# iden3/wasmsnark

Measured on AMD Instinct MI355X. Metric: BN128 Groth16 prove ms @ 2^20 constraints, lower is better.
Workload: dtype u256 (Montgomery; 9x29-bit limbs, v_mad_u64_u32); 1 GPU; BN128 full Groth16 prove, synthetic 2^20-constraint R1CS (1-3 non-zeros per column of A and B, every variable present), key and witness resident in HBM, r and s injected; parallelism=1 GPU, no collective, lanes=2, device=AMD Radeon Graphics gfx950:sramecc+:xnack- CUs=256 device=0

## Files before the change

wasmsnark_amd/csrc/internal.h:

```cpp
#pragma once
#include <atomic>
#include <condition_variable>
#include <functional>
#include <map>
#include <memory>
#include <mutex>
#include <thread>
#include <vector>

#include "curve.h"
#include "curve_pair.h"
#include "rt.h"

namespace wsnark {

struct KernelTimer {
    bool enabled = false;
    bool dominant_only = false;
    std::mutex mu;
    unsigned long generation = 0;
    struct Rec { const char* name; hipEvent_t a, b; };
    std::vector<Rec> recs;
    std::vector<hipEvent_t> pool;
    std::map<std::string, std::pair<double, uint64_t>> acc;
// ... 118 lines not shown
void warm_fixedbase(hipStream_t s);
void context_join_warm(Context* C);
#define WS_DEFINE_WARM(tu) \
    __global__ void warm_kernel_##tu(int) {} \
    void warm_##tu(hipStream_t s) { hipLaunchKernelGGL(warm_kernel_##tu, dim3(1), dim3(64), 0, s, 0); (void)hipGetLastError(); }

struct LaneLock {
    Lane* L = nullptr;
    Context* C = nullptr;
    std::unique_lock<std::mutex> lk;
    LaneLock() {}
    LaneLock(LaneLock&& o) : L(o.L), C(o.C), lk(std::move(o.lk)) { o.L = nullptr; o.C = nullptr; }
    LaneLock(const LaneLock&) = delete;
    LaneLock& operator=(const LaneLock&) = delete;
    ~LaneLock();
    Lane* operator->() const { return L; }
    Lane& operator*() const { return *L; }
};
LaneLock acquire_lane(Context* C);

int upload_staged(void* d_dst, const void* h_src, size_t bytes, hipStream_t s);
typedef std::function<int(size_t, size_t, hipStream_t)> ChunkFn;
int upload_pipelined(void* d_dst, const void* h_src, size_t bytes, hipStream_t s, const ChunkFn& on_chunk, bool* direct_out = nullptr);

long tuning_get(const char* name, long dflt);
double tuning_get_real(const char* name, double dflt);
void tuning_set(const char* name, long value);

int ntt_dev(Lane& L, Fe* d_data, uint64_t n, int odd, int inverse, hipStream_t s, uint64_t count = 1);
struct NttRowCoset { const Fe* lo; const Fe* hi; uint32_t hc, shift, row0, row_mask; };
struct NttRowPost { Fe* out; const Fe* lo; const Fe* hi; uint32_t h, lr1, lr2, k; uint64_t row0; };
struct NttRowGather { const Fe* in; uint32_t lr1, lr2, k; };
int ntt_run(Lane& L, const Fe* d_src, const Fe* d_in2, Fe* d_dst, const Fe* combine_e, uint64_t n, int odd, int inverse,
            hipStream_t s, uint64_t count = 1, const NttRowCoset* rc_pre = nullptr, const NttRowPost* rc_post = nullptr,
            const struct NttRowGather* rc_gather = nullptr);
int ntt_coset_tables_kernel_format(int bits, const Fe** lo, const Fe** hi, uint32_t* hc, hipStream_t s);
int ntt_twiddle_tables(int bits, int inverse, const Fe** lo, const Fe** hi, int* h, hipStream_t s, bool internal = false);

int ntt_coset_tables(int bits, const Fe** lo, const Fe** hi, int* hc, Fe* n_inv, hipStream_t s);

int msm_g1_dev(Lane& L, const Fe* d_scalars, const Affine<Fq>* d_points, uint64_t n, WindowShard sh, Jac<Fq>* out_host, hipStream_t s);
int msm_g2_dev(Lane& L, const Fe* d_scalars, const Affine<Fq2>* d_points, uint64_t n, WindowShard sh, Jac<Fq2>* out_host, hipStream_t s);
int msm_g1_host(Lane& L, const void* h_scalars, const void* h_points, uint64_t n, WindowShard sh, Jac<Fq>* out_host);
int msm_g2_host(Lane& L, const void* h_scalars, const void* h_points, uint64_t n, WindowShard sh, Jac<Fq2>* out_host);
int msm_plan_dev(Lane& L, const Fe* d_scalars, uint64_t n, WindowShard sh, hipStream_t s, uint32_t table_c = 0);
int msm_plan_begin(Lane& L, uint64_t n, WindowShard sh, hipStream_t s, uint32_t table_c = 0);
int msm_plan_count(Lane& L, const Fe* d_scalars, uint64_t i0, uint64_t i1, hipStream_t s);
int msm_plan_finish(Lane& L, const Fe* d_scalars, hipStream_t s);
uint32_t msm_table_rows(uint32_t table_c);
uint32_t msm_table_window(uint64_t n);
int msm_build_table(int which, void* d_table, uint64_t n, uint32_t table_c, hipStream_t s, void* d_tmp = nullptr, size_t tmp_bytes = 0);
size_t msm_table_scratch_bytes(uint64_t lanes);
int msm_points_mask(const Affine<Fq>* d_g1, const Affine<Fq2>* d_g2, uint64_t n, uint8_t* d_mask, uint32_t* skipped_host, hipStream_t s);
int msm_g1_launch(Lane& L, const Affine<Fq>* d_points, bool prepared, int* slot, hipStream_t s);
int msm_g2_launch(Lane& L, const Affine<Fq2>* d_points, bool prepared, int* slot, hipStream_t s);
int msm_g1_launch_batch(Lane& L, const Affine<Fq>* const* d_points, int nsets, bool prepared, int* slots, hipStream_t s, const int* plan_ids = nullptr);
int msm_g1_launch_acc_only(Lane& L, const Affine<Fq>* d_points, bool prepared, int* slot, hipStream_t s);
int msm_g1_launch_tail_merged(Lane& L, int slot_a, int slot_b, hipStream_t s, bool* merged);
void msm_select_plan(Lane& L, int id);
int msm_plan_variant(Lane& L, int src_id, int dst_id, const uint8_t* d_mask, hipStream_t s);
static const uint32_t kMsmPlanInfoWords = 24;
int selftest_msm_plan(Lane& L, const void* h_scalars, uint64_t n, uint32_t table_c, WindowShard sh, const uint8_t* h_mask,
                      uint32_t* info, uint32_t* bstart, uint32_t* bend, uint64_t cap_buckets, uint32_t* vals, uint64_t cap_vals,
                      uint32_t* tasks, uint64_t cap_tasks, uint32_t* multi, uint64_t cap_multi, uint32_t* hot, uint64_t cap_hot);
bool msm_ready(Lane& L, int slot);
int msm_g1_finish(Lane& L, int slot, XYZZ<Fq>* out_host);
int msm_g2_finish(Lane& L, int slot, XYZZ<Fq2>* out_host);
void msm_abort_slots(Lane& L, const int* slots, int nslots, hipStream_t a, hipStream_t b);
void msm_workspace_free(Lane& L);
int msm_prepare_points(int which, void* d_points, uint64_t n, hipStream_t s);

int groth16_verify(const uint8_t* vk, size_t vk_len, const uint8_t* inputs, uint64_t n_inputs, const uint8_t* proof384, int* valid);
struct PairConsts;
int pairing_consts(const PairConsts** out);
int groth16_verify_batch(const uint8_t* vk, size_t vk_len, const void* inputs, uint64_t n_inputs, const void* proofs384, uint64_t count,
                         uint8_t* status_host, bool on_device, hipStream_t s);
int points_codec(int g, bool compress, const void* in, uint64_t n, int enc, uint32_t flags, void* out, uint8_t* status, uint64_t* n_bad);
int proofs_codec(bool compress, const void* in, uint64_t count, int enc, void* out, uint8_t* status);
int groth16_verify_batch_compressed(const uint8_t* vk, size_t vk_len, const void* inputs, uint64_t n_inputs, const void* proofs128, uint64_t count,
                                    int enc, uint8_t* status_host, bool on_device, hipStream_t stream);

struct CsrMatrix {
    uint32_t n_rows = 0;
    uint32_t n_cols = 0;
    uint64_t nnz = 0;
    DevBuf row_ptr;
    DevBuf col;
    DevBuf coef;
};
int pols_to_csr(const uint8_t* pols, size_t len, uint32_t n_signals, uint32_t domain, CsrMatrix* out,
                size_t* consumed, hipStream_t s, void (*release)(const void* p, size_t n) = nullptr);
int scan_exclusive_dev(const uint32_t* d_in, uint32_t n, uint32_t* d_tiles, uint32_t* d_out, uint32_t* d_cursor, hipStream_t s);
int calc_h_dev(Lane& L, const Fe* d_signals_plain, uint32_t n_signals, const CsrMatrix& A, const CsrMatrix& B,
               uint32_t domain, Fe* d_h_out, hipStream_t s);
int fr_map_dev(const Fe* d_in, Fe* d_out, uint64_t n, int to_mont, hipStream_t s);
int fr_mul_dev(const Fe* d_a, const Fe* d_b, Fe* d_out, uint64_t n, hipStream_t s);
int eval_ab_dev(Lane& L, const Fe* d_signals_plain, uint32_t n_signals, const CsrMatrix& A, const CsrMatrix& B, uint32_t domain,
                Fe* d_a, Fe* d_b, hipStream_t s);
int dist_combine_dev(const Fe* d_e, const Fe* d_o, Fe* d_h, uint64_t rows, uint64_t cols, uint64_t row0, uint32_t log_n1, uint32_t log_n, hipStream_t s);
int dist_scale_dev(Fe* d_data, uint64_t stack, uint64_t rows, uint64_t cols, uint64_t row0, uint32_t log_n1, uint32_t log_n, int mode, int inverse, hipStream_t s);

struct KeySections {
    uint32_t n_vars, n_public, domain;
    const uint8_t *alfa1, *beta1, *delta1, *beta2, *delta2;
    const uint8_t* polsA; uint64_t lenA;
    const uint8_t* polsB; uint64_t lenB;
    const uint8_t *A, *B1, *B2, *Cpts, *H;
    uint64_t lenPA, lenPB1, lenPB2, lenPC, lenPH;
    void (*release)(const void* p, size_t n) = nullptr;
// ... 99 lines not shown
```

wasmsnark_amd/csrc/msm.hip:

```cpp
#include <string.h>

#include <algorithm>
#include <chrono>

#include "internal.h"
namespace wsnark {

#ifndef WS_ACC_WAVES
#define WS_ACC_WAVES 3
#endif
#ifndef WS_ACC_WAVES_G2
#define WS_ACC_WAVES_G2 2
#endif
#ifndef WS_G2_PREFETCH
#define WS_G2_PREFETCH 0
#endif
#ifndef WS_G1_PREFETCH
#define WS_G1_PREFETCH 1
#endif
#ifndef WS_MADD_WIDE
#define WS_MADD_WIDE 1
#endif
static const uint32_t CHUNK = 8;
#ifndef WS_TAIL_L2_DEFAULT
// ... 886 lines not shown
    const uint32_t slot = threadIdx.x / IO::LPP, nslots = blockDim.x / IO::LPP;
    const uint32_t in_row = r == w_row ? logJ + 2 : r <= logJ ? r : logJ + 1;
    const uint32_t bit = (r > logJ && r != w_row) ? r - logJ - 1 : 0xFFFFFFFFu;
    typename C::Pt acc = C::infinity();
    for (uint32_t v = slot; v < P; v += nslots)
        if (bit == 0xFFFFFFFFu || ((v >> bit) & 1u)) acc = C::add(acc, IO::load(rows, ((uint64_t)g * P + v) * nsum_in + in_row));
    IO::store(sh, slot, acc);
    __syncthreads();
    for (uint32_t step = nslots >> 1; step >= 1; step >>= 1) {
        if (slot < step) IO::store(sh, slot, C::add(IO::load(sh, slot), IO::load(sh, slot + step)));
        __syncthreads();
    }
    if (slot == 0) IO::store_ref(out, (uint64_t)g * nrows_out + r, IO::load(sh, 0));
}


static uint32_t pick_window(uint64_t n) {
    { const long c = tuning_get("MSM_C", 0); if (c >= 4 && c <= 16) return (uint32_t)c; }
    int lg = 0;
    while (((uint64_t)1 << (lg + 1)) <= n) lg++;
    int c = lg - 4;
    if (c < 4) c = 4;
    if (c > 16) c = 16;
    return (uint32_t)c;
}

struct MsmPlanInfo {
    uint64_t n = 0;
    uint32_t c = 0, W = 0, NB = 0, nbuckets = 0, m = 0, J = 0, logJ = 0, nsum = 0, lmax = 0, hot_cap = 0;
    uint32_t hot_min = 1024;
    uint32_t ps_lo_bits = 0, ps_idx_bits = 0, ps_nbins = 0, ps_bthr = 0;
    uint32_t ps_HB = 0, ps_tile = 0, ps_thr = 0;
    bool ps_valid = false, ps_e32 = false;
    bool building = false;
    uint32_t Wall = 0, w_off = 0, w_stride = 1;
    bool flat = false;
    uint32_t tW = 0, tNB = 0;
    uint32_t tP = 1, groups = 1, nrows = 0;
    bool reduce = false;
    uint32_t m1 = 0, m2 = 1, J1 = 0;
    uint32_t ntasks = 0, nmulti = 0;
    bool valid = false;
};
struct MsmPending {
    bool active = false;
    int which = 0;
    int plan_id = 0;
    MsmPlanInfo info;
    DevBuf d_sums, d_rows;
    MsmScratch S;
    void* h_sums = nullptr;
    size_t h_bytes = 0;
    hipEvent_t ev = nullptr;
    const void* d_points_used = nullptr;
    int partner = -1;
    void release() {
        if (h_sums) (void)hipHostFree(h_sums);
        if (ev) (void)hipEventDestroy(ev);
        h_sums = nullptr; ev = nullptr; h_bytes = 0; active = false;
        d_sums.release(); d_rows.release();
        S.buckets.release(); S.partials.release(); S.chunkS.release(); S.chunkA.release(); S.points_conv.release(); S.hot_sums.release();
        S.hot_done.release(); S.tree_half.release(); S.tree_done.release();
    }
};

static const int kPlans = 4;
static const int kPendingSlots = 8;
struct MsmWorkspace {
    struct Plan { MsmPlanInfo info; MsmScratch S; } plan[kPlans];
    int cur = 0;
    MsmPending slot[kPendingSlots];
    hipEvent_t host_ev = nullptr;
    hipEvent_t conv_ev[2] = {nullptr, nullptr};
    DevBuf conv_buf;
};
static MsmWorkspace& ws(Lane& L) {
    if (!L.msm) L.msm = new MsmWorkspace();
    return *L.msm;
}
void msm_workspace_free(Lane& L) {
    if (!L.msm) return;
    MsmWorkspace& M = *L.msm;
    if (M.host_ev) (void)hipEventDestroy(M.host_ev);
    for (auto& e : M.conv_ev) if (e) (void)hipEventDestroy(e);
    for (auto& p : M.slot) p.release();
    delete L.msm;
    L.msm = nullptr;
}
void msm_select_plan(Lane& L, int id) { ws(L).cur = (id >= 0 && id < kPlans) ? id : 0; }

void msm_abort_slots(Lane& L, const int* slots, int nslots, hipStream_t a, hipStream_t b) {
    if (a) (void)hipStreamSynchronize(a);
    if (b && b != a) (void)hipStreamSynchronize(b);
    if (!L.msm) return;
    for (int k = 0; k < nslots; k++)
        if (slots[k] >= 0 && slots[k] < kPendingSlots) L.msm->slot[slots[k]].active = false;
}

template <class H>
static int msm_finish_t(MsmPending& P, typename H::Pt* out_host) {
    typedef typename H::Pt HPt;
    const MsmPlanInfo& I = P.info;
    if (I.n == 0) { *out_host = H::infinity(); P.active = false; return WS_OK; }
    struct Done { MsmPending& p; ~Done() { p.active = false; } } done{P};
    const bool trace = tuning_get("TRACE", 0) == 1;
    const auto t_wait = std::chrono::steady_clock::now();
    WS_HIP_CHECK(hipEventSynchronize(P.ev));
    const auto t_tail = std::chrono::steady_clock::now();
    const HPt* sums = reinterpret_cast<const HPt*>(P.h_sums);
    if (I.flat && I.reduce) {
        uint32_t logm = 0, logt = 0, logP = 0;
        while ((1u << logm) < I.m) logm++;
        while ((1u << logt) < I.tNB) logt++;
        while ((1u << logP) < I.tP) logP++;
        HPt acc = H::infinity();
        for (int q = (int)I.logJ - 1; q >= 0; q--) acc = H::add(H::dbl(acc), sums[q]);
        if (I.m2 > 1) {
            uint32_t logm1 = 0;
            while ((1u << logm1) < I.m1) logm1++;
            for (uint32_t k = logm1; k < logm; k++) acc = H::dbl(acc);
            acc = H::add(acc, sums[I.logJ + 1 + logP]);
            for (uint32_t k = 0; k < logm1; k++) acc = H::dbl(acc);
        } else {
            for (uint32_t k = 0; k < logm; k++) acc = H::dbl(acc);
        }
        acc = H::add(acc, sums[I.logJ]);
        HPt tot = H::infinity();
        for (int pb = (int)logP - 1; pb >= 0; pb--) tot = H::add(H::dbl(tot), sums[I.logJ + 1 + (uint32_t)pb]);
        for (uint32_t k = 0; k < logt; k++) tot = H::dbl(tot);
        *out_host = H::add(acc, tot);
        if (trace)
            fprintf(stderr, "[wsnark trace]   msm finish (%s, table, rows folded on the GPU): waited %.3f ms for the GPU, host tail %.3f ms\n", sizeof(HPt) > 128 ? "G2" : "G1",
                    std::chrono::duration<double, std::milli>(t_tail - t_wait).count(),
                    std::chrono::duration<double, std::milli>(std::chrono::steady_clock::now() - t_tail).count());
        return WS_OK;
    }
    if (I.flat) {
        uint32_t logm = 0, logt = 0;
        while ((1u << logm) < I.m) logm++;
        while ((1u << logt) < I.tNB) logt++;
        HPt acc = H::infinity();
        for (int q = (int)I.logJ - 1; q >= 0; q--) {
            acc = H::dbl(acc);
            for (uint32_t v = 0; v < I.tW; v++) acc = H::add(acc, sums[(size_t)v * I.nsum + q]);
        }
        for (uint32_t k = 0; k < logm; k++) acc = H::dbl(acc);
// ... 402 lines not shown
    MsmScratch& S = P.S;
    WS_HIP_CHECK(S.buckets.reserve((size_t)nbuckets * sizeof(Pt)));
    WS_HIP_CHECK(S.partials.reserve((size_t)I.hot_cap * sizeof(Pt)));
    WS_HIP_CHECK(S.chunkS.reserve(((size_t)W * I.J1 + (I.m2 > 1 ? (size_t)2 * W * J : 0)) * sizeof(Pt)));
    WS_HIP_CHECK(S.chunkA.reserve(((size_t)W * I.J1 + (I.m2 > 1 ? (size_t)W * J : 0)) * sizeof(Pt)));
    const size_t sums_bytes = (I.reduce ? (size_t)I.groups * I.nrows : (size_t)W * nsum) * sizeof(Pt);
    WS_HIP_CHECK(P.d_sums.reserve(sums_bytes));
    if (I.reduce) WS_HIP_CHECK(P.d_rows.reserve((size_t)W * nsum * sizeof(Pt)));
    WS_HIP_CHECK(S.tree_half.reserve((size_t)W * 6 * sizeof(Pt)));
    {
        const size_t db = (size_t)W * 3 * sizeof(uint32_t);
        if (!S.tree_done.p || S.tree_done.bytes < db) { WS_HIP_CHECK(S.tree_done.alloc(db)); WS_HIP_CHECK(hipMemsetAsync(S.tree_done.p, 0, db, s)); }
    }
    if (P.h_bytes < sums_bytes) {
        if (P.h_sums) (void)hipHostFree(P.h_sums);
        P.h_sums = nullptr; P.h_bytes = 0;
        WS_HIP_CHECK(hipHostMalloc(&P.h_sums, sums_bytes, 0));
        P.h_bytes = sums_bytes;
    }
    if (!P.ev) WS_HIP_CHECK(hipEventCreate(&P.ev));
    WS_HIP_CHECK(S.hot_sums.reserve(((size_t)I.hot_cap / HOT_SLICE + (size_t)I.hot_cap / I.hot_min + 32) * sizeof(Pt)));
    {
        const size_t hot_bytes = ((size_t)I.hot_cap / I.hot_min + 16) * 4;
        if (!S.hot_done.p || S.hot_done.bytes < hot_bytes) { WS_HIP_CHECK(S.hot_done.alloc(hot_bytes)); WS_HIP_CHECK(hipMemsetAsync(S.hot_done.p, 0, hot_bytes, s)); }
    }

    KernelTimer& T = X->timer;
    if (I.flat && !prepared) { set_last_error("msm: a table plan needs a prepared fixed-base table"); return WS_ERR_ARG; }
    if (C::Field::kInternalDomain && !prepared) {
        WS_HIP_CHECK(S.points_conv.reserve((size_t)n * sizeof(typename C::AffP)));
        T.begin("msm_convert_points", s);
        hipLaunchKernelGGL(msm_convert_points<C>, dim3(ceil_div_u64(n, 256)), dim3(256), 0, s, d_points,
                           S.points_conv.as<typename C::AffP>(), n);
        T.end(s);
        d_points = S.points_conv.as<typename C::AffP>();
    }
    P.d_points_used = d_points;
    if (!defer_kernels) {
        MsmPending* one[1] = {&P};
        int rc = msm_acc_sets<C>(L, one, 1, which, s);
        if (rc) return rc;
    }
    P.active = true;
    *slot_out = slot;
    return WS_OK;
}

template <class C> struct TailCurve { typedef C type; typedef C paired; };
template <> struct TailCurve<G1R29> { typedef G1R29I type; typedef G1P29 paired; };
template <> struct TailCurve<G2R29> { typedef G2P29 type; typedef G2Q29 paired; };
static bool tail_pair_g1() { return tuning_get("TAIL_PAIR_G1", 1) != 0; }
static bool tail_quad_g2() { return tuning_get("TAIL_QUAD_G2", 1) != 0; }
template <class C> static bool tail_split() { return sizeof(typename C::AffP) > 64 ? tail_quad_g2() : tail_pair_g1(); }
template <class C, class CC = C>
static int msm_launch_tail(Lane& L, const int* slot_ids, int nslots, hipStream_t s, int second_slot = -1) {
    typedef PointIO<C> IO;
    typedef typename IO::Stored St;
    static_assert(sizeof(typename PointIO<CC>::Stored) == sizeof(St), "the chunk and tree kernels share their buffers");
    Context* X = ctx();
    if (!s) s = L.stream;
    MsmPending* slots = ws(L).slot;
    const MsmPlanInfo& I = slots[slot_ids[0]].info;
    if (I.n == 0) return WS_OK;
    TailSets<C> ts;
    for (int k = 0; k < 4; k++) {
        MsmPending& P = slots[slot_ids[k < nslots ? k : 0]];
        ts.buckets[k] = P.S.buckets.template as<St>();
        ts.l1S[k] = P.S.chunkS.template as<St>();
        ts.l1A[k] = P.S.chunkA.template as<St>();
        ts.chunkS[k] = P.S.chunkS.template as<St>() + (I.m2 > 1 ? (size_t)I.tW * I.J1 : 0);
        ts.chunkA[k] = P.S.chunkA.template as<St>() + (I.m2 > 1 ? (size_t)I.tW * I.J1 : 0);
        ts.chunkW[k] = P.S.chunkS.template as<St>() + (size_t)I.tW * I.J1 + (size_t)I.tW * I.J;
        ts.rows[k] = P.d_rows.template as<St>();
        ts.sums[k] = P.d_sums.template as<St>();
        ts.bstart[k] = ws(L).plan[P.plan_id].S.bstart.template as<uint32_t>();
        ts.bend[k] = ws(L).plan[P.plan_id].S.bend.template as<uint32_t>();
        ts.half[k] = P.S.tree_half.template as<St>();
        ts.half_done[k] = P.S.tree_done.template as<uint32_t>();
        ts.buckets2[k] = nullptr; ts.bstart2[k] = ts.bend2[k] = nullptr;
        if (second_slot >= 0) {
            MsmPending& P2 = slots[second_slot];
            ts.buckets2[k] = P2.S.buckets.template as<St>();
            ts.bstart2[k] = ws(L).plan[P2.plan_id].S.bstart.template as<uint32_t>();
            ts.bend2[k] = ws(L).plan[P2.plan_id].S.bend.template as<uint32_t>();
        }
    }
    const uint32_t J = I.J, logJ = I.logJ, nsum = I.nsum, LPP = IO::LPP, W = I.tW;
    KernelTimer& T = X->timer;
    T.begin("msm_chunks", s);
    {
        TailSets<CC> tc;
        static_assert(sizeof tc == sizeof ts, "same pointers");
        memcpy(&tc, &ts, sizeof tc);
        for (int k = 0; k < 4; k++) { tc.chunkS[k] = const_cast<typename PointIO<CC>::Stored*>(tc.l1S[k]); tc.chunkA[k] = const_cast<typename PointIO<CC>::Stored*>(tc.l1A[k]); }
        const dim3 grid(ceil_div_u64((uint64_t)W * I.J1 * PointIO<CC>::LPP, 256), nslots);
        if (second_slot >= 0) hipLaunchKernelGGL((msm_chunks<CC, true>), grid, dim3(256), 0, s, tc, W * I.J1, I.m1);
        else hipLaunchKernelGGL((msm_chunks<CC, false>), grid, dim3(256), 0, s, tc, W * I.J1, I.m1);
    }
    T.end(s);
    WS_HIP_CHECK(hipGetLastError());
    if (I.m2 > 1) {
        T.begin("msm_chunks2", s);
        hipLaunchKernelGGL(msm_chunks2<C>, dim3(ceil_div_u64((uint64_t)2 * W * J * LPP, 256), nslots), dim3(256), 0, s, ts, W * J, I.m2);
        T.end(s);
        WS_HIP_CHECK(hipGetLastError());
    }
    uint32_t tslots = 1;
    const uint32_t tree_wgs = (logJ + 2 * (nsum - logJ)) * W * (uint32_t)nslots;
    const uint32_t smax = ((LPP == 1 || TreeBound<C>::value >= 1024) && tree_wgs <= 256) ? 512 : 256;
    while (tslots < (J > 1 ? J / 2 : 1) && tslots < smax && tslots * LPP < (uint32_t)TreeBound<C>::value) tslots <<= 1;
    T.begin("msm_tree", s);
    hipLaunchKernelGGL(msm_tree<C>, dim3(logJ + 2 * (nsum - logJ), W, nslots), dim3(tslots * LPP), (size_t)tslots * sizeof(St), s, ts, J, logJ, I.reduce ? 0u : 1u,
                       nsum);
    T.end(s);
    WS_HIP_CHECK(hipGetLastError());
    size_t sums_bytes;
    if (I.reduce) {
        uint32_t rslots = 1;
        while (rslots < I.tP && rslots < smax && rslots * LPP < (uint32_t)TreeBound<C>::value) rslots <<= 1;
        T.begin("msm_rows", s);
        hipLaunchKernelGGL(msm_rows<C>, dim3(I.nrows, I.groups, nslots), dim3(rslots * LPP), (size_t)rslots * sizeof(St), s, ts, I.tP, logJ, nsum, I.nrows, I.m2 > 1 ? I.nrows - 1 : 0xFFFFFFFFu);
        T.end(s);
        WS_HIP_CHECK(hipGetLastError());
        sums_bytes = (size_t)I.groups * I.nrows * sizeof(St);
    } else {
        sums_bytes = (size_t)W * nsum * sizeof(St);
    }
    for (int k = 0; k < nslots; k++) {
        MsmPending& P = slots[slot_ids[k]];
        WS_HIP_CHECK(hipMemcpyAsync(P.h_sums, P.d_sums.p, sums_bytes, hipMemcpyDeviceToHost, s));
        WS_HIP_CHECK(hipEventRecord(P.ev, s));
    }
    if (second_slot >= 0) WS_HIP_CHECK(hipEventRecord(slots[second_slot].ev, s));
    return WS_OK;
}

template <class C, class H>
static int msm_launch(Lane& L, int which, const typename H::Aff* d_points_ref, bool prepared, int* slot_out, hipStream_t s) {
    if (!s) s = L.stream;
    int rc = msm_launch_acc<C, H>(L, which, d_points_ref, prepared, slot_out, s);
    if (rc) return rc;
    rc = tail_split<C>() ? msm_launch_tail<typename TailCurve<C>::paired, typename TailCurve<C>::type>(L, slot_out, 1, s)
                         : msm_launch_tail<typename TailCurve<C>::type>(L, slot_out, 1, s);
    if (rc) msm_abort_slots(L, slot_out, 1, s, nullptr);
    return rc;
}

int msm_g1_launch_batch(Lane& L, const Affine<Fq>* const* d_points, int nsets, bool prepared, int* slots, hipStream_t s, const int* plan_ids) {
    if (!ctx()) return WS_ERR_NOINIT;
    if (nsets < 1 || nsets > 4) return WS_ERR_ARG;
    if (!s) s = L.stream;
    MsmWorkspace& M = ws(L);
    const int keep = M.cur;
    for (int k = 0; k < nsets; k++) slots[k] = -1;
    int rc = WS_OK;
    const MsmPlanInfo& I0 = M.plan[plan_ids ? plan_ids[0] : M.cur].info;
    const bool batched = nsets > 1 && I0.valid && I0.n && I0.nbuckets <= (1u << 16);
    for (int k = 0; k < nsets && !rc; k++) {
        if (plan_ids) msm_select_plan(L, plan_ids[k]);
        rc = msm_launch_acc<G1R29, G1>(L, 0, d_points[k], prepared, &slots[k], s, batched);
        if (plan_ids) msm_select_plan(L, keep);
    }
    if (!rc && batched) {
        MsmPending* Ps[4];
        for (int k = 0; k < nsets; k++) Ps[k] = &M.slot[slots[k]];
        rc = msm_acc_sets<G1R29>(L, Ps, nsets, 0, s);
    }
    if (!rc) rc = tail_pair_g1() ? msm_launch_tail<TailCurve<G1R29>::paired, TailCurve<G1R29>::type>(L, slots, nsets, s)
                                 : msm_launch_tail<TailCurve<G1R29>::type>(L, slots, nsets, s);
    if (rc) msm_abort_slots(L, slots, nsets, s, nullptr);
    return rc;
}

int msm_g1_launch(Lane& L, const Affine<Fq>* d_points, bool prepared, int* slot, hipStream_t s) {
    if (!ctx()) return WS_ERR_NOINIT;
    return msm_launch<G1R29, G1>(L, 0, d_points, prepared, slot, s);
}
int msm_g1_launch_acc_only(Lane& L, const Affine<Fq>* d_points, bool prepared, int* slot, hipStream_t s) {
    if (!ctx()) return WS_ERR_NOINIT;
    if (!s) s = L.stream;
    return msm_launch_acc<G1R29, G1>(L, 0, d_points, prepared, slot, s);
}
static bool msm_tail_mergeable(const MsmPlanInfo& a, const MsmPlanInfo& b) {
    return a.n && b.n && a.flat && b.flat && a.c == b.c && a.W == b.W && a.Wall == b.Wall && a.w_off == b.w_off && a.w_stride == b.w_stride &&
           a.NB == b.NB && a.nbuckets == b.nbuckets && a.tNB == b.tNB && a.tP == b.tP && a.tW == b.tW && a.groups == b.groups &&
           a.m1 == b.m1 && a.m2 == b.m2 && a.m == b.m && a.J1 == b.J1 && a.J == b.J && a.logJ == b.logJ && a.nsum == b.nsum &&
           a.nrows == b.nrows && a.reduce == b.reduce;
}
int msm_g1_launch_tail_merged(Lane& L, int slot_a, int slot_b, hipStream_t s, bool* merged) {
    if (!ctx()) return WS_ERR_NOINIT;
    if (!s) s = L.stream;
    *merged = false;
    if (!L.msm || slot_a < 0 || slot_b < 0 || slot_a >= kPendingSlots || slot_b >= kPendingSlots || slot_a == slot_b) return WS_ERR_ARG;
    MsmPending &A = L.msm->slot[slot_a], &B = L.msm->slot[slot_b];
    if (!A.active || !B.active || A.which != 0 || B.which != 0) return WS_ERR_ARG;
    int rc = WS_OK;
    if (msm_tail_mergeable(A.info, B.info)) {
        rc = tail_pair_g1() ? msm_launch_tail<TailCurve<G1R29>::paired, TailCurve<G1R29>::type>(L, &slot_a, 1, s, slot_b)
                            : msm_launch_tail<TailCurve<G1R29>::type>(L, &slot_a, 1, s, slot_b);
        if (!rc) { A.partner = slot_b; *merged = true; }
    } else {
        for (const int* one : {&slot_a, &slot_b}) {
            if (rc) break;
            rc = tail_pair_g1() ? msm_launch_tail<TailCurve<G1R29>::paired, TailCurve<G1R29>::type>(L, one, 1, s)
                                : msm_launch_tail<TailCurve<G1R29>::type>(L, one, 1, s);
        }
    }
    return rc;
}
int msm_g2_launch(Lane& L, const Affine<Fq2>* d_points, bool prepared, int* slot, hipStream_t s) {
    if (!ctx()) return WS_ERR_NOINIT;
    return msm_launch<G2R29, G2>(L, 1, d_points, prepared, slot, s);
}
static MsmPending* live_slot(Lane& L, int slot, int which) {
    if (!L.msm || slot < 0 || slot >= kPendingSlots) return nullptr;
    MsmPending& P = L.msm->slot[slot];
    return (P.active && (which < 0 || P.which == which)) ? &P : nullptr;
}
bool msm_ready(Lane& L, int slot) {
    MsmPending* P = live_slot(L, slot, -1);
    return P && (P->info.n == 0 || (P->ev && hipEventQuery(P->ev) == hipSuccess));
}
int msm_g1_finish(Lane& L, int slot, XYZZ<Fq>* out_host) {
    MsmPending* P = live_slot(L, slot, 0);
    if (!P) return WS_ERR_ARG;
    const int partner = P->partner;
    P->partner = -1;
    const int rc = msm_finish_t<G1>(*P, out_host);
    if (partner >= 0) L.msm->slot[partner].active = false;
    return rc;
}
int msm_g2_finish(Lane& L, int slot, XYZZ<Fq2>* out_host) {
    MsmPending* P = live_slot(L, slot, 1);
    return P ? msm_finish_t<G2>(*P, out_host) : WS_ERR_ARG;
}

__global__ __launch_bounds__(256) void msm_points_mask_kernel(const Affine<Fq>* __restrict__ g1, const Affine<Fq2>* __restrict__ g2,
                                                                uint64_t n, uint8_t* __restrict__ mask, uint32_t* __restrict__ skipped) {
    const uint64_t i = (uint64_t)blockIdx.x * blockDim.x + threadIdx.x;
    if (i >= n) return;
    bool inf = true;
    if (g1) inf = inf && Fq::is_zero(g1[i].x);
    if (g2) inf = inf && Fq::is_zero(g2[i].x.c0) && Fq::is_zero(g2[i].x.c1);
    mask[i] = inf ? 0 : 1;
    if (inf) atomicAdd(skipped, 1u);
}
int msm_points_mask(const Affine<Fq>* d_g1, const Affine<Fq2>* d_g2, uint64_t n, uint8_t* d_mask, uint32_t* skipped_host, hipStream_t s) {
    Context* X = ctx();
    if (!X) return WS_ERR_NOINIT;
    if (!s) s = X->stream;
    *skipped_host = 0;
    if (n == 0) return WS_OK;
    DevBuf cnt;
    WS_HIP_CHECK(cnt.alloc(4));
    WS_HIP_CHECK(hipMemsetAsync(cnt.p, 0, 4, s));
    hipLaunchKernelGGL(msm_points_mask_kernel, dim3(ceil_div_u64(n, 256)), dim3(256), 0, s, d_g1, d_g2, n, d_mask, cnt.as<uint32_t>());
    WS_HIP_CHECK(hipGetLastError());
    WS_HIP_CHECK(hipMemcpyAsync(skipped_host, cnt.p, 4, hipMemcpyDeviceToHost, s));
    WS_HIP_CHECK(hipStreamSynchronize(s));
    return WS_OK;
}

int msm_prepare_points(int which, void* d_points, uint64_t n, hipStream_t s) {
    Context* X = ctx();
    if (!X) return WS_ERR_NOINIT;
// ... 270 lines not shown
```

wasmsnark_amd/csrc/prove.hip:

```cpp
#include <errno.h>
#include <fcntl.h>
#include <stdio.h>
#include <string.h>
#include <sys/syscall.h>
#include <unistd.h>

#include <atomic>
#include <chrono>
#include <future>

#include <functional>
#include <thread>

#include "internal.h"
#include "keybytes.h"

namespace wsnark {


static int pkey_table_state(ProvingKey* K, bool wait, uint32_t* cw, uint32_t* ch) {
    *cw = K->table_cw; *ch = K->table_ch;
    if (!K->table_cw && !K->table_ch) return WS_OK;
    int st = K->tables_ready.load(std::memory_order_acquire);
#ifdef WSNARK_EMUL
// ... 345 lines not shown
    hipStream_t s2 = overlap ? L.stream2 : s;
    int slots[5] = {-1, -1, -1, -1, -1};
    int &hA = slots[0], &hB1 = slots[1], &hC = slots[2], &hB2 = slots[3], &hH = slots[4];
    struct Abort {
        Lane& L; int* slots; hipStream_t a, b; bool armed;
        ~Abort() { if (armed) { msm_select_plan(L, 0); if (L.stream3) (void)hipStreamSynchronize(L.stream3); msm_abort_slots(L, slots, 5, a, b); } }
    } guard{L, slots, s, s2, true};
    for (hipEvent_t* e : {&L.ev_start, &L.ev_h})
        if (!*e) WS_HIP_CHECK(hipEventCreateWithFlags(e, hipEventDisableTiming));
    msm_select_plan(L, 0);
    if (h_witness) {
        hipStream_t sc = L.stream_copy;
        for (hipEvent_t* e : {&L.ev_chunk[0], &L.ev_chunk[1]})
            if (!*e) WS_HIP_CHECK(hipEventCreateWithFlags(e, hipEventDisableTiming));
        WS_HIP_CHECK(hipEventRecord(L.ev_start, s));
        WS_HIP_CHECK(hipStreamWaitEvent(sc, L.ev_start, 0));
        if ((rc = msm_plan_begin(L, nv, sh, s, table_cw))) return rc;
        unsigned k = 0;
        const uint64_t lo_sig = K->lo, hi_sig = (uint64_t)K->lo + nv;
        rc = upload_pipelined(const_cast<Fe*>(d_witness_all), h_witness, (size_t)K->n_vars * 32, sc, [&](size_t blo, size_t bhi, hipStream_t cq) -> int {
            hipEvent_t ev = L.ev_chunk[k++ & 1];
            WS_HIP_CHECK(hipEventRecord(ev, cq));
            WS_HIP_CHECK(hipStreamWaitEvent(s, ev, 0));
            uint64_t e0 = blo / 32, e1 = bhi / 32;
            if (e0 < lo_sig) e0 = lo_sig;
            if (e1 > hi_sig) e1 = hi_sig;
            return e0 < e1 ? msm_plan_count(L, d_witness, e0 - lo_sig, e1 - lo_sig, s) : (int)WS_OK;
        });
        if (rc) return rc;
        tr.mark("witness staged, histogram enqueued per chunk");
        WS_HIP_CHECK(hipEventRecord(L.ev_start, s));
        if ((rc = msm_plan_finish(L, d_witness, s))) return rc;
    } else {
        WS_HIP_CHECK(hipEventRecord(L.ev_start, s));
        if ((rc = msm_plan_dev(L, d_witness, nv, sh, s, table_cw))) return rc;
    }
    Fe* d_h = nullptr;
    bool calc_h_done = false;
    auto enqueue_calc_h = [&]() -> int {
        if (s2 != s) WS_HIP_CHECK(hipStreamWaitEvent(s2, L.ev_start, 0));
        WS_HIP_CHECK(L.h.reserve((size_t)dom * 32));
        d_h = L.h.as<Fe>();
        int r = calc_h ? calc_h(s2, d_h) : calc_h_dev(L, d_witness_all, K->n_vars, K->polsA, K->polsB, dom, d_h, s2);
        calc_h_done = true;
        return r;
    };
    if (!skip_h && !calc_h && s2 != s) {
        if ((rc = enqueue_calc_h())) return rc;
        tr.mark("calc_h enqueued");
    }
    int planA = 0, planB = 0;
    if (K->sparseB && msm_plan_variant(L, 0, 2, K->maskB.as<uint8_t>(), s) == WS_OK) planB = 2;
    if (K->sparseA && msm_plan_variant(L, 0, 3, K->maskA.as<uint8_t>(), s) == WS_OK) planA = 3;
    const bool small = overlap && (uint64_t)nv * msm_table_rows(table_cw ? table_cw : 16) < ((uint64_t)1 << 23) && L.stream3 && s != L.stream3;
    const long ch_sw = tuning_get("PROVE_CH_TAIL", 2);
    const bool ch_merge = one_call && !skip_h && !calc_h && sh.off == 0 && sh.stride == 1 && K->shard_world == 1 && !K->h_log_m && table_cw &&
                          table_cw == table_ch && nv && K->h_local && (ch_sw == 1 || (ch_sw != 0 && !small));
    const Affine<Fq>* g1sets[3] = {K->pointsA.as<Affine<Fq>>(), K->pointsB1.as<Affine<Fq>>(), K->pointsC.as<Affine<Fq>>()};
    const int plans[3] = {planA, planB, 0};
    int g1slots[3] = {-1, -1, -1};
    if (small) {
        hipStream_t s3 = L.stream3;
        for (hipEvent_t* e : {&L.ev_plan, &L.ev_g2})
            if (!*e) WS_HIP_CHECK(hipEventCreateWithFlags(e, hipEventDisableTiming));
        WS_HIP_CHECK(hipEventRecord(L.ev_plan, s));
        WS_HIP_CHECK(hipStreamWaitEvent(s3, L.ev_plan, 0));
        msm_select_plan(L, planB);
        rc = msm_g2_launch(L, K->pointsB2.as<Affine<Fq2>>(), true, &hB2, s3);
        msm_select_plan(L, 0);
        if (rc) return rc;
        WS_HIP_CHECK(hipEventRecord(L.ev_g2, s3));
        rc = msm_g1_launch_batch(L, g1sets, ch_merge ? 2 : 3, true, g1slots, s, plans);
        hA = g1slots[0]; hB1 = g1slots[1]; hC = g1slots[2];
        if (rc) return rc;
        if (ch_merge && (rc = msm_g1_launch_acc_only(L, K->pointsC.as<Affine<Fq>>(), true, &hC, s))) return rc;
        WS_HIP_CHECK(hipStreamWaitEvent(s, L.ev_g2, 0));
        tr.mark("plan(w) + B2 on queue 3 + A, B1, C batched");
    } else {
        msm_select_plan(L, planB);
        rc = msm_g2_launch(L, K->pointsB2.as<Affine<Fq2>>(), true, &hB2, s);
        msm_select_plan(L, 0);
        if (rc) return rc;
        tr.mark("plan(w) [+ variants] + launch B2");
        rc = msm_g1_launch_batch(L, g1sets, 2, true, g1slots, s, plans);
        hA = g1slots[0]; hB1 = g1slots[1];
        if (rc) return rc;
        msm_select_plan(L, 0);
        rc = ch_merge ? msm_g1_launch_acc_only(L, K->pointsC.as<Affine<Fq>>(), true, &hC, s)
                      : msm_g1_launch(L, K->pointsC.as<Affine<Fq>>(), true, &hC, s);
        if (rc) return rc;
        tr.mark("launch A, B1, C");
    }
    if (skip_h) {
        if ((rc = msm_g1_finish(L, hA, &out->A))) return rc;
        if ((rc = msm_g1_finish(L, hB1, &out->B1))) return rc;
        if (after_ab1) after_ab1(*out);
        if ((rc = msm_g1_finish(L, hC, &out->C))) return rc;
        if ((rc = msm_g2_finish(L, hB2, &out->B2))) return rc;
        out->H = G1::infinity();
        guard.armed = false;
        return WS_OK;
    }
    if (!calc_h_done) {
        if ((rc = enqueue_calc_h())) return rc;
        tr.mark("calc_h enqueued");
    }
    msm_select_plan(L, (s2 != s || ch_merge) ? 1 : 0);
    rc = msm_plan_dev(L, d_h + K->hlo, K->h_local, sh, s2, table_ch);
    if (!rc) rc = ch_merge ? msm_g1_launch_acc_only(L, K->pointsH.as<Affine<Fq>>(), true, &hH, s2)
                           : msm_g1_launch(L, K->pointsH.as<Affine<Fq>>(), true, &hH, s2);
    msm_select_plan(L, 0);
    if (rc) return rc;
    if (s2 != s) { WS_HIP_CHECK(hipEventRecord(L.ev_h, s2)); WS_HIP_CHECK(hipStreamWaitEvent(s, L.ev_h, 0)); }
    bool ch_merged = false;
    if (ch_merge && (rc = msm_g1_launch_tail_merged(L, hC, hH, s, &ch_merged))) return rc;
    tr.mark(ch_merged ? "plan(h) + accumulate H + one tail for C + H" : "plan(h) + launch H");
    const bool g2_fin = !small;
    if (g2_fin && (rc = msm_g2_finish(L, hB2, &out->B2))) return rc;
    if ((rc = msm_g1_finish(L, hA, &out->A))) return rc;
    if ((rc = msm_g1_finish(L, hB1, &out->B1))) return rc;
    tr.mark(g2_fin ? "finish B2, A, B1" : "finish A, B1");
    if (after_ab1) after_ab1(*out);
    if (ch_merged) {
        if ((rc = msm_g1_finish(L, hC, &out->C))) return rc;
        out->H = G1::infinity();
        if (!g2_fin && (rc = msm_g2_finish(L, hB2, &out->B2))) return rc;
        tr.mark(g2_fin ? "finish C + H" : "finish C + H, B2");
        guard.armed = false;
        return WS_OK;
    }
    if (!g2_fin && !ch_merge && (rc = msm_g1_finish(L, hC, &out->C))) return rc;
    tr.mark(g2_fin ? "host work on A, B1" : "host work on A, B1; finish C");
    {
        const int hX = g2_fin ? hC : hB2;
        auto finish_x = [&]() -> int { return g2_fin ? msm_g1_finish(L, hC, &out->C) : msm_g2_finish(L, hB2, &out->B2); };
        bool doneX = false, doneH = false;
        for (unsigned spins = 0; !(doneX && doneH); spins++) {
            if (!doneX && (doneH || msm_ready(L, hX))) { if ((rc = finish_x())) return rc; doneX = true; continue; }
            if (!doneH && (doneX || msm_ready(L, hH))) { if ((rc = msm_g1_finish(L, hH, &out->H))) return rc; doneH = true; continue; }
            if (spins > 64) std::this_thread::yield();
            if (spins > (1u << 22)) {
                if (!doneH) { if ((rc = msm_g1_finish(L, hH, &out->H))) return rc; doneH = true; }
                if (!doneX) { if ((rc = finish_x())) return rc; doneX = true; }
            }
        }
    }
    if (!g2_fin && ch_merge && (rc = msm_g1_finish(L, hC, &out->C))) return rc;
    tr.mark(g2_fin ? "finish H, C" : "finish H, B2");
    guard.armed = false;
    return WS_OK;
}

struct Blinding {
    Fe rr, ss, rs;
    struct Pre { G1::Pt r_delta1, s_delta1, rs_delta1; G2::Pt s_delta2; };
    std::future<Pre> pre;
    const uint8_t* rb() const { return reinterpret_cast<const uint8_t*>(&rr); }
    const uint8_t* sb() const { return reinterpret_cast<const uint8_t*>(&ss); }
    ~Blinding() { if (pre.valid()) pre.wait(); }
};

static thread_local uint8_t t_last_rs[64];
static thread_local bool t_have_rs = false;
bool last_blinding(uint8_t* r32, uint8_t* s32) {
    if (!t_have_rs) return false;
    if (r32) memcpy(r32, t_last_rs, 32);
    if (s32) memcpy(s32, t_last_rs + 32, 32);
    return true;
// ... 307 lines not shown
```

Baseline: 8.874 ms.

## Run MSM tail reduction levels on side stream to overlap with accumulation

Splits the MSM tail into a chunk stage and a levels (tree/reduction) stage, and lets the levels stage run on a third stream after an event dependency on the chunk stage. In the prover, the B2 and A/B1 tails in the non-small path are routed to stream3 so their reductions overlap with later accumulation work (C, H) on the main streams, with a join before finishing. This adds event record/wait overhead and contention between concurrent kernels for CUs, and abort now also synchronizes stream3.

```diff
diff --git a/wasmsnark_amd/csrc/internal.h b/wasmsnark_amd/csrc/internal.h
--- a/wasmsnark_amd/csrc/internal.h
+++ b/wasmsnark_amd/csrc/internal.h
@@ -194,9 +194,11 @@
 int msm_build_table(int which, void* d_table, uint64_t n, uint32_t table_c, hipStream_t s, void* d_tmp = nullptr, size_t tmp_bytes = 0);
 size_t msm_table_scratch_bytes(uint64_t lanes);
 int msm_points_mask(const Affine<Fq>* d_g1, const Affine<Fq2>* d_g2, uint64_t n, uint8_t* d_mask, uint32_t* skipped_host, hipStream_t s);
-int msm_g1_launch(Lane& L, const Affine<Fq>* d_points, bool prepared, int* slot, hipStream_t s);
-int msm_g2_launch(Lane& L, const Affine<Fq2>* d_points, bool prepared, int* slot, hipStream_t s);
-int msm_g1_launch_batch(Lane& L, const Affine<Fq>* const* d_points, int nsets, bool prepared, int* slots, hipStream_t s, const int* plan_ids = nullptr);
+int msm_g1_launch(Lane& L, const Affine<Fq>* d_points, bool prepared, int* slot, hipStream_t s, hipStream_t s_levels = nullptr);
+int msm_g2_launch(Lane& L, const Affine<Fq2>* d_points, bool prepared, int* slot, hipStream_t s, hipStream_t s_levels = nullptr);
+int msm_g1_launch_batch(Lane& L, const Affine<Fq>* const* d_points, int nsets, bool prepared, int* slots, hipStream_t s, const int* plan_ids = nullptr,
+                        hipStream_t s_levels = nullptr);
+long msm_tail_side_switch();
 int msm_g1_launch_acc_only(Lane& L, const Affine<Fq>* d_points, bool prepared, int* slot, hipStream_t s);
 int msm_g1_launch_tail_merged(Lane& L, int slot_a, int slot_b, hipStream_t s, bool* merged);
 void msm_select_plan(Lane& L, int id);
diff --git a/wasmsnark_amd/csrc/msm.hip b/wasmsnark_amd/csrc/msm.hip
--- a/wasmsnark_amd/csrc/msm.hip
+++ b/wasmsnark_amd/csrc/msm.hip
@@ -962,12 +962,14 @@
     void* h_sums = nullptr;
     size_t h_bytes = 0;
     hipEvent_t ev = nullptr;
+    hipEvent_t ev_chunks = nullptr;
     const void* d_points_used = nullptr;
     int partner = -1;
     void release() {
         if (h_sums) (void)hipHostFree(h_sums);
         if (ev) (void)hipEventDestroy(ev);
-        h_sums = nullptr; ev = nullptr; h_bytes = 0; active = false;
+        if (ev_chunks) (void)hipEventDestroy(ev_chunks);
+        h_sums = nullptr; ev = ev_chunks = nullptr; h_bytes = 0; active = false;
         d_sums.release(); d_rows.release();
         S.buckets.release(); S.partials.release(); S.chunkS.release(); S.chunkA.release(); S.points_conv.release(); S.hot_sums.release();
         S.hot_done.release(); S.tree_half.release(); S.tree_done.release();
@@ -1002,6 +1004,7 @@
 void msm_abort_slots(Lane& L, const int* slots, int nslots, hipStream_t a, hipStream_t b) {
     if (a) (void)hipStreamSynchronize(a);
     if (b && b != a) (void)hipStreamSynchronize(b);
+    if (L.stream3 && L.stream3 != a && L.stream3 != b) (void)hipStreamSynchronize(L.stream3);
     if (!L.msm) return;
     for (int k = 0; k < nslots; k++)
         if (slots[k] >= 0 && slots[k] < kPendingSlots) L.msm->slot[slots[k]].active = false;
@@ -1510,17 +1513,11 @@
 static bool tail_pair_g1() { return tuning_get("TAIL_PAIR_G1", 1) != 0; }
 static bool tail_quad_g2() { return tuning_get("TAIL_QUAD_G2", 1) != 0; }
 template <class C> static bool tail_split() { return sizeof(typename C::AffP) > 64 ? tail_quad_g2() : tail_pair_g1(); }
-template <class C, class CC = C>
-static int msm_launch_tail(Lane& L, const int* slot_ids, int nslots, hipStream_t s, int second_slot = -1) {
-    typedef PointIO<C> IO;
-    typedef typename IO::Stored St;
-    static_assert(sizeof(typename PointIO<CC>::Stored) == sizeof(St), "the chunk and tree kernels share their buffers");
-    Context* X = ctx();
-    if (!s) s = L.stream;
+template <class C>
+static void tail_sets(Lane& L, const int* slot_ids, int nslots, int second_slot, TailSets<C>& ts) {
+    typedef typename PointIO<C>::Stored St;
     MsmPending* slots = ws(L).slot;
     const MsmPlanInfo& I = slots[slot_ids[0]].info;
-    if (I.n == 0) return WS_OK;
-    TailSets<C> ts;
     for (int k = 0; k < 4; k++) {
         MsmPending& P = slots[slot_ids[k < nslots ? k : 0]];
         ts.buckets[k] = P.S.buckets.template as<St>();
@@ -1543,7 +1540,18 @@
             ts.bend2[k] = ws(L).plan[P2.plan_id].S.bend.template as<uint32_t>();
         }
     }
-    const uint32_t J = I.J, logJ = I.logJ, nsum = I.nsum, LPP = IO::LPP, W = I.tW;
+}
+template <class C, class CC = C>
+static int msm_launch_tail_chunks(Lane& L, const int* slot_ids, int nslots, hipStream_t s, int second_slot = -1) {
+    typedef typename PointIO<C>::Stored St;
+    static_assert(sizeof(typename PointIO<CC>::Stored) == sizeof(St), "the chunk and tree kernels share their buffers");
+    Context* X = ctx();
+    if (!s) s = L.stream;
+    const MsmPlanInfo& I = ws(L).slot[slot_ids[0]].info;
+    if (I.n == 0) return WS_OK;
+    TailSets<C> ts;
+    tail_sets<C>(L, slot_ids, nslots, second_slot, ts);
+    const uint32_t W = I.tW;
     KernelTimer& T = X->timer;
     T.begin("msm_chunks", s);
     {
@@ -1557,6 +1565,21 @@
     }
     T.end(s);
     WS_HIP_CHECK(hipGetLastError());
+    return WS_OK;
+}
+template <class C>
+static int msm_launch_tail_levels(Lane& L, const int* slot_ids, int nslots, hipStream_t s, int second_slot = -1) {
+    typedef PointIO<C> IO;
+    typedef typename IO::Stored St;
+    Context* X = ctx();
+    if (!s) s = L.stream;
+    MsmPending* slots = ws(L).slot;
+    const MsmPlanInfo& I = slots[slot_ids[0]].info;
+    if (I.n == 0) return WS_OK;
+    TailSets<C> ts;
+    tail_sets<C>(L, slot_ids, nslots, second_slot, ts);
+    const uint32_t J = I.J, logJ = I.logJ, nsum = I.nsum, LPP = IO::LPP, W = I.tW;
+    KernelTimer& T = X->timer;
     if (I.m2 > 1) {
         T.begin("msm_chunks2", s);
         hipLaunchKernelGGL(msm_chunks2<C>, dim3(ceil_div_u64((uint64_t)2 * W * J * LPP, 256), nslots), dim3(256), 0, s, ts, W * J, I.m2);
@@ -1592,22 +1615,44 @@
     if (second_slot >= 0) WS_HIP_CHECK(hipEventRecord(slots[second_slot].ev, s));
     return WS_OK;
 }
+long msm_tail_side_switch() { return tuning_get("PROVE_TAIL_SIDE", 2); }
+static hipStream_t tail_levels_queue(Lane& L, hipStream_t s, hipStream_t s_levels) {
+    if (s_levels) return s_levels;
+    return (msm_tail_side_switch() == 1 && L.stream3 && s != L.stream3) ? L.stream3 : s;
+}
+template <class C, class CC = C>
+static int msm_launch_tail(Lane& L, const int* slot_ids, int nslots, hipStream_t s, int second_slot = -1, hipStream_t s_levels = nullptr) {
+    if (!s) s = L.stream;
+    int rc = msm_launch_tail_chunks<C, CC>(L, slot_ids, nslots, s, second_slot);
+    if (rc) return rc;
+    MsmPending& P0 = ws(L).slot[slot_ids[0]];
+    if (s_levels && s_levels != s && P0.info.n) {
+        if (!P0.ev_chunks) WS_HIP_CHECK(hipEventCreateWithFlags(&P0.ev_chunks, hipEventDisableTiming));
+        WS_HIP_CHECK(hipEventRecord(P0.ev_chunks, s));
+        WS_HIP_CHECK(hipStreamWaitEvent(s_levels, P0.ev_chunks, 0));
+    } else {
+        s_levels = s;
+    }
+    return msm_launch_tail_levels<C>(L, slot_ids, nslots, s_levels, second_slot);
+}
 
 template <class C, class H>
-static int msm_launch(Lane& L, int which, const typename H::Aff* d_points_ref, bool prepared, int* slot_out, hipStream_t s) {
+static int msm_launch(Lane& L, int which, const typename H::Aff* d_points_ref, bool prepared, int* slot_out, hipStream_t s, hipStream_t s_levels) {
     if (!s) s = L.stream;
+    s_levels = tail_levels_queue(L, s, s_levels);
     int rc = msm_launch_acc<C, H>(L, which, d_points_ref, prepared, slot_out, s);
     if (rc) return rc;
-    rc = tail_split<C>() ? msm_launch_tail<typename TailCurve<C>::paired, typename TailCurve<C>::type>(L, slot_out, 1, s)
-                         : msm_launch_tail<typename TailCurve<C>::type>(L, slot_out, 1, s);
+    rc = tail_split<C>() ? msm_launch_tail<typename TailCurve<C>::paired, typename TailCurve<C>::type>(L, slot_out, 1, s, -1, s_levels)
+                         : msm_launch_tail<typename TailCurve<C>::type>(L, slot_out, 1, s, -1, s_levels);
     if (rc) msm_abort_slots(L, slot_out, 1, s, nullptr);
     return rc;
 }
 
-int msm_g1_launch_batch(Lane& L, const Affine<Fq>* const* d_points, int nsets, bool prepared, int* slots, hipStream_t s, const int* plan_ids) {
+int msm_g1_launch_batch(Lane& L, const Affine<Fq>* const* d_points, int nsets, bool prepared, int* slots, hipStream_t s, const int* plan_ids, hipStream_t s_levels) {
     if (!ctx()) return WS_ERR_NOINIT;
     if (nsets < 1 || nsets > 4) return WS_ERR_ARG;
     if (!s) s = L.stream;
+    s_levels = tail_levels_queue(L, s, s_levels);
     MsmWorkspace& M = ws(L);
     const int keep = M.cur;
     for (int k = 0; k < nsets; k++) slots[k] = -1;
@@ -1624,15 +1669,15 @@
         for (int k = 0; k < nsets; k++) Ps[k] = &M.slot[slots[k]];
         rc = msm_acc_sets<G1R29>(L, Ps, nsets, 0, s);
     }
-    if (!rc) rc = tail_pair_g1() ? msm_launch_tail<TailCurve<G1R29>::paired, TailCurve<G1R29>::type>(L, slots, nsets, s)
-                                 : msm_launch_tail<TailCurve<G1R29>::type>(L, slots, nsets, s);
+    if (!rc) rc = tail_pair_g1() ? msm_launch_tail<TailCurve<G1R29>::paired, TailCurve<G1R29>::type>(L, slots, nsets, s, -1, s_levels)
+                                 : msm_launch_tail<TailCurve<G1R29>::type>(L, slots, nsets, s, -1, s_levels);
     if (rc) msm_abort_slots(L, slots, nsets, s, nullptr);
     return rc;
 }
 
-int msm_g1_launch(Lane& L, const Affine<Fq>* d_points, bool prepared, int* slot, hipStream_t s) {
+int msm_g1_launch(Lane& L, const Affine<Fq>* d_points, bool prepared, int* slot, hipStream_t s, hipStream_t s_levels) {
     if (!ctx()) return WS_ERR_NOINIT;
-    return msm_launch<G1R29, G1>(L, 0, d_points, prepared, slot, s);
+    return msm_launch<G1R29, G1>(L, 0, d_points, prepared, slot, s, s_levels);
 }
 int msm_g1_launch_acc_only(Lane& L, const Affine<Fq>* d_points, bool prepared, int* slot, hipStream_t s) {
     if (!ctx()) return WS_ERR_NOINIT;
@@ -1666,9 +1711,9 @@
     }
     return rc;
 }
-int msm_g2_launch(Lane& L, const Affine<Fq2>* d_points, bool prepared, int* slot, hipStream_t s) {
+int msm_g2_launch(Lane& L, const Affine<Fq2>* d_points, bool prepared, int* slot, hipStream_t s, hipStream_t s_levels) {
     if (!ctx()) return WS_ERR_NOINIT;
-    return msm_launch<G2R29, G2>(L, 1, d_points, prepared, slot, s);
+    return msm_launch<G2R29, G2>(L, 1, d_points, prepared, slot, s, s_levels);
 }
 static MsmPending* live_slot(Lane& L, int slot, int which) {
     if (!L.msm || slot < 0 || slot >= kPendingSlots) return nullptr;
diff --git a/wasmsnark_amd/csrc/prove.hip b/wasmsnark_amd/csrc/prove.hip
--- a/wasmsnark_amd/csrc/prove.hip
+++ b/wasmsnark_amd/csrc/prove.hip
@@ -421,7 +421,18 @@
     int planA = 0, planB = 0;
     if (K->sparseB && msm_plan_variant(L, 0, 2, K->maskB.as<uint8_t>(), s) == WS_OK) planB = 2;
     if (K->sparseA && msm_plan_variant(L, 0, 3, K->maskA.as<uint8_t>(), s) == WS_OK) planA = 3;
-    const bool small = overlap && (uint64_t)nv * msm_table_rows(table_cw ? table_cw : 16) < ((uint64_t)1 << 23) && L.stream3 && s != L.stream3;
+    const bool small = overlap && (uint64_t)nv * msm_table_rows(table_cw ? table_cw : 16) < ((uint64_t)1 << 23) && L.stream3 && s != L.stream3 &&
+                       tuning_get("PROVE_FULL_SIZE", 0) != 1;
+    const long side_sw = msm_tail_side_switch();
+    const bool side = overlap && L.stream3 && s != L.stream3 && s2 != L.stream3 && (side_sw == 1 || (side_sw != 0 && !small));
+    hipStream_t s_side = side ? L.stream3 : s;
+    if (side && !L.ev_tail) WS_HIP_CHECK(hipEventCreateWithFlags(&L.ev_tail, hipEventDisableTiming));
+    auto join_side = [&]() -> int {
+        if (!side) return WS_OK;
+        WS_HIP_CHECK(hipEventRecord(L.ev_tail, L.stream3));
+        WS_HIP_CHECK(hipStreamWaitEvent(s, L.ev_tail, 0));
+        return WS_OK;
+    };
     const long ch_sw = tuning_get("PROVE_CH_TAIL", 2);
     const bool ch_merge = one_call && !skip_h && !calc_h && sh.off == 0 && sh.stride == 1 && K->shard_world == 1 && !K->h_log_m && table_cw &&
                           table_cw == table_ch && nv && K->h_local && (ch_sw == 1 || (ch_sw != 0 && !small));
@@ -435,11 +446,11 @@
         WS_HIP_CHECK(hipEventRecord(L.ev_plan, s));
         WS_HIP_CHECK(hipStreamWaitEvent(s3, L.ev_plan, 0));
         msm_select_plan(L, planB);
-        rc = msm_g2_launch(L, K->pointsB2.as<Affine<Fq2>>(), true, &hB2, s3);
+        rc = msm_g2_launch(L, K->pointsB2.as<Affine<Fq2>>(), true, &hB2, s3, s3);
         msm_select_plan(L, 0);
         if (rc) return rc;
         WS_HIP_CHECK(hipEventRecord(L.ev_g2, s3));
-        rc = msm_g1_launch_batch(L, g1sets, ch_merge ? 2 : 3, true, g1slots, s, plans);
+        rc = msm_g1_launch_batch(L, g1sets, ch_merge ? 2 : 3, true, g1slots, s, plans, s_side);
         hA = g1slots[0]; hB1 = g1slots[1]; hC = g1slots[2];
         if (rc) return rc;
         if (ch_merge && (rc = msm_g1_launch_acc_only(L, K->pointsC.as<Affine<Fq>>(), true, &hC, s))) return rc;
@@ -447,20 +458,21 @@
         tr.mark("plan(w) + B2 on queue 3 + A, B1, C batched");
     } else {
         msm_select_plan(L, planB);
-        rc = msm_g2_launch(L, K->pointsB2.as<Affine<Fq2>>(), true, &hB2, s);
+        rc = msm_g2_launch(L, K->pointsB2.as<Affine<Fq2>>(), true, &hB2, s, s_side);
         msm_select_plan(L, 0);
         if (rc) return rc;
         tr.mark("plan(w) [+ variants] + launch B2");
-        rc = msm_g1_launch_batch(L, g1sets, 2, true, g1slots, s, plans);
+        rc = msm_g1_launch_batch(L, g1sets, 2, true, g1slots, s, plans, s_side);
         hA = g1slots[0]; hB1 = g1slots[1];
         if (rc) return rc;
         msm_select_plan(L, 0);
         rc = ch_merge ? msm_g1_launch_acc_only(L, K->pointsC.as<Affine<Fq>>(), true, &hC, s)
-                      : msm_g1_launch(L, K->pointsC.as<Affine<Fq>>(), true, &hC, s);
+                      : msm_g1_launch(L, K->pointsC.as<Affine<Fq>>(), true, &hC, s, s);
         if (rc) return rc;
         tr.mark("launch A, B1, C");
     }
     if (skip_h) {
+        if ((rc = join_side())) return rc;
         if ((rc = msm_g1_finish(L, hA, &out->A))) return rc;
         if ((rc = msm_g1_finish(L, hB1, &out->B1))) return rc;
         if (after_ab1) after_ab1(*out);
@@ -477,12 +489,13 @@
     msm_select_plan(L, (s2 != s || ch_merge) ? 1 : 0);
     rc = msm_plan_dev(L, d_h + K->hlo, K->h_local, sh, s2, table_ch);
     if (!rc) rc = ch_merge ? msm_g1_launch_acc_only(L, K->pointsH.as<Affine<Fq>>(), true, &hH, s2)
-                           : msm_g1_launch(L, K->pointsH.as<Affine<Fq>>(), true, &hH, s2);
+                           : msm_g1_launch(L, K->pointsH.as<Affine<Fq>>(), true, &hH, s2, s2);
     msm_select_plan(L, 0);
     if (rc) return rc;
     if (s2 != s) { WS_HIP_CHECK(hipEventRecord(L.ev_h, s2)); WS_HIP_CHECK(hipStreamWaitEvent(s, L.ev_h, 0)); }
     bool ch_merged = false;
     if (ch_merge && (rc = msm_g1_launch_tail_merged(L, hC, hH, s, &ch_merged))) return rc;
+    if ((rc = join_side())) return rc;
     tr.mark(ch_merged ? "plan(h) + accumulate H + one tail for C + H" : "plan(h) + launch H");
     const bool g2_fin = !small;
     if (g2_fin && (rc = msm_g2_finish(L, hB2, &out->B2))) return rc;
```

Result: faster. 8.616 ms (median of 6 runs) (-2.9%).
